# prequel-dev/plz4

Hardware: AMD Instinct MI355X
Metric: MiB/s enc+dec, 4MiB independent blocks, level 1, block-checksum on (duplex steps over 2 streams) (higher is better)
Workload: dtype u8

## Files before the change

plz4_amd/_native.py:

```python
from __future__ import annotations

import ctypes as C
import os

import numpy as np

HERE = os.path.dirname(os.path.abspath(__file__))
LIB_PATH = os.path.join(HERE, "libplz4hip.so")

ABI_VERSION = 2
SYMBOLS = [
    "plz4hip_abi_version", "plz4hip_device_count", "plz4hip_ctx_create", "plz4hip_ctx_destroy",
    "plz4hip_last_error", "plz4hip_compress_bound", "plz4hip_compress_batch", "plz4hip_decompress_batch",
    "plz4hip_xxh32_batch", "plz4hip_encode_records", "plz4hip_decode_records", "plz4hip_dev_stage_stride",
    "plz4hip_dev_encode_records", "plz4hip_dev_compact_records", "plz4hip_dev_scatter_records",
    "plz4hip_dev_decode_records", "plz4hip_dev_decode_records_ex", "plz4hip_dev_duplex_records", "plz4hip_dev_encode_body", "plz4hip_dev_duplex_body", "plz4hip_dev_encode_records_ex", "plz4hip_dev_encode_body_ex", "plz4hip_dev_compress", "plz4hip_dev_decompress", "plz4hip_ctx_trim",
    "plz4hip_ctx_counters",
    "plz4hip_dev_resident_waves", "plz4hip_dict_create", "plz4hip_dict_destroy", "plz4hip_compress_batch_dict", "plz4hip_decode_records_chains",
    "plz4hip_decompress_batch_dict", "plz4hip_encode_records_ex", "plz4hip_decode_records_ex",
    "plz4hip_xxh32_stream_create", "plz4hip_xxh32_stream_destroy", "plz4hip_xxh32_stream_reset", "plz4hip_xxh32_stream_update",
    "plz4hip_dev_xxh32_stream_update", "plz4hip_xxh32_stream_sum", "plz4hip_ctx_set_content_hash",
    "plz4hip_mgpu_create", "plz4hip_mgpu_destroy", "plz4hip_mgpu_count", "plz4hip_mgpu_ctx", "plz4hip_mgpu_last_error",
    "plz4hip_mgpu_compress_batch", "plz4hip_mgpu_decompress_batch", "plz4hip_mgpu_encode_records", "plz4hip_mgpu_decode_records",
    "plz4hip_mgpu_dev_encode_frame", "plz4hip_mgpu_dev_decode_frame",
# ... 408 lines not shown
        self._chk(self.L.plz4hip_dev_xxh32_stream_update(self.h, h, ptr, n, stream))

    def hash_sum(self, h) -> int:
        out = C.c_uint32()
        self._chk(self.L.plz4hip_xxh32_stream_sum(self.h, h, C.byref(out)))
        return int(out.value)

    def set_content_hash(self, h):
        self._chk(self.L.plz4hip_ctx_set_content_hash(self.h, h))

    def trim(self):
        self._chk(self.L.plz4hip_ctx_trim(self.h))

    COUNTERS = ("fx_blocks", "fx_rounds_last", "fx_pieces_again", "dx_blocks", "dxl_blocks", "dxl_rounds_last", "dxl_groups_last",
                "fxl_blocks", "l1x_blocks", "hcx_blocks", "dx_big_blocks", "dx_big_rounds_last", "dx_big_runs_last",
                "mx_blocks", "mx_rounds_last", "mx_pieces_again", "mxl_blocks", "hb_blocks", "hb_pieces_last")

    def counters(self) -> dict:
        out = (C.c_int64 * len(self.COUNTERS))()
        rc = int(self.L.plz4hip_ctx_counters(self.h, out, len(self.COUNTERS)))
        if rc < 0:
            self._chk(rc)
        return {k: int(out[i]) for i, k in enumerate(self.COUNTERS)}


class MultiEngine:

    def __init__(self, devices):
        self.L = load()
        arr = (C.c_int * len(devices))(*devices)
        h = C.c_void_p()
# ... 73 lines not shown
```

plz4_amd/csrc/plz4hip.hip:

```cpp
#include <hip/hip_runtime.h>

#include <array>
#include <atomic>
#include <mutex>
#include <thread>
#include <string>
#include <vector>
#include <cstdio>
#include <cstring>

#include "../../include/plz4hip.h"
#include "stream_ws.h"
#if defined(PLZ4_STATS)
__device__ unsigned long long plz4_stats[24];
#endif
#include "lz4_device.inl"
#include "lz4_seq_device.inl"
#include "lz4hc_device.inl"
#include "lz4hc12_device.inl"
#include "lz4hc_lists_device.inl"
#include "lz4hc_lazy_device.inl"
#include "lz4hcx_device.inl"
#include "lz4_dx_device.inl"
#include "lz4_fx_device.inl"
// ... 42 lines not shown
    int             h12Gather, h12Idle;
    SeqInfo*        l1Info;
    uint64_t*       l1Seq;      int64_t l1SeqStride;
    uint32_t*       l1ChunkBytes; uint32_t* l1ChunkOff; int l1MaxChunks;
    uint8_t*        l1Bk;
    int             l1MaxLen;
    int             lzSegs, lzMinSeg;
    uint64_t*       lzRec;      uint64_t* lzBridge;  int64_t lzRecStride;
    LzSegMeta*      lzMeta;     uint64_t* lzStarts;  LzPiece* lzPieces;
    uint64_t*       dxT;        int64_t dxTStride;
    uint32_t*       dxPtr;      int64_t dxPtrStride;
    DxUnit*         dxUnits;    int dxMaxSeg;   int dxRound;
    DxInfo*         dxInfo;
    int64_t*        bodyOff;    int64_t bodyCap;
    uint32_t*       gate;       uint32_t gateSeq;
    const int64_t*  dxSrcOff;   const int32_t* dxLen;
    int32_t*        dxHashBad;
    int32_t*        dxlFirst;   int32_t* dxlChain;   uint32_t* dxlMoved;   int32_t* dxlGood;   int dxlRounds;
    int32_t*        dxlDead;    int dxlBlk0;    int dxlGroup;   int dxlGroups;
    uint64_t*       dxbTG;      int64_t dxbTGStride;   DxbEntry* dxbEnt;   int dxbGroups;   int dxbG;
    DxRun*          dxbRuns;    int dxbRunRoom;   int dxbThr;   DxbInfo* dxbInfo;   int dxbRounds;
};

__device__ __forceinline__ int next_block(uint32_t* q)
{
    uint32_t v = 0;
    if ((threadIdx.x & 63u) == 0) v = atomicAdd(q, 1u);
    return (int)plz4_readfirstlane(v);
}

// ... 50 lines not shown
        const uint8_t* s = a.src + (int64_t)i * a.srcStride;
        encode_out(a, i, s, n, false, [&](uint8_t* out, int cap) { return wave_encode_block(s, n, out, cap, lds); });
    }
}

template <int kLdsWin = 0>
__device__ __forceinline__ void l1_parse_loop(const CodecArgs& a, uint32_t* lds, uint8_t* scr = nullptr)
{
    for (int i = next_block(a.queue); i < a.nBlocks; i = next_block(a.queue)) {
        const int gi = a.blk0 + i;
        const int n  = block_len(a, gi);
        int lastAnchor = 0, nseq = -1;
        if (n >= 0 && n <= a.l1MaxLen)
            nseq = wave_parse_l1<kLdsWin>(a.src + (int64_t)gi * a.srcStride, n, lds, a.l1Seq + (int64_t)i * a.l1SeqStride, &lastAnchor, scr);
        if ((threadIdx.x & 63u) == 0) { SeqInfo inf; inf.nseq = nseq; inf.lastAnchor = lastAnchor; inf.total = 0; inf.stored = 0; a.l1Info[i] = inf; }
    }
    if (a.gate && (threadIdx.x & 63u) == 0) atomicMax(a.gate, a.gateSeq);
}
__global__ __launch_bounds__(64) void k_parse_gate(const uint32_t* gate, uint32_t want)
{
    for (int it = 0; it < 400000; ++it) {
        if ((int32_t)(__hip_atomic_load(gate, __ATOMIC_RELAXED, __HIP_MEMORY_SCOPE_AGENT) - want) >= 0) break;
        __builtin_amdgcn_s_sleep(127);
    }
}
template <int W> __global__ __launch_bounds__(64 * W) void k_l1_parse(CodecArgs a)
{
    ENC_WAVE_TABLE(lds);
    l1_parse_loop<2>(a, lds);
}

template <bool kBack, bool kSeg = false> __device__ __forceinline__ void l1_sizes_body(const CodecArgs a, const FxlBlk* xb = nullptr)
{
    const int i = blockIdx.y, wave = blockIdx.x * 4 + (int)(threadIdx.x >> 6), nW = gridDim.x * 4;
    const int nseq = a.l1Info[i].nseq;
    if (nseq <= 0) return;
    const int gi = a.blk0 + i;
    const uint8_t*  s   = a.src + (int64_t)gi * a.srcStride;
    const uint64_t* seq = a.l1Seq + (int64_t)i * a.l1SeqStride;
    const int nChunks = (nseq + kSeqChunk - 1) / kSeqChunk;
    for (int c = wave; c < nChunks; c += nW) {
        const uint32_t v = seq_emit_sizes<kBack, kSeg>(s, seq, kBack ? a.l1Bk + (int64_t)i * a.l1SeqStride : nullptr, nseq, c, kSeg ? max_(xb[i].pfx, 0) : 0);
        if ((threadIdx.x & 63u) == 0) a.l1ChunkBytes[(int64_t)i * a.l1MaxChunks + c] = v;
    }
}
template <bool kBack> __global__ __launch_bounds__(256) void k_l1_sizes(CodecArgs a) { l1_sizes_body<kBack>(a); }

__global__ __launch_bounds__(256) void k_l1_scan(CodecArgs a)
{
    const int i = blockIdx.x * 4 + (int)(threadIdx.x >> 6);
    if (i >= a.nBlocks) return;
    const int gi = a.blk0 + i;
    const int n  = block_len(a, gi);
    SeqInfo inf = a.l1Info[i];
    const int cap = a.rawMode ? cap_of(a, gi) : a.bsz;
    int total = 0;
    const bool broken = inf.nseq == kSeqEngineFailed;
    if (inf.nseq >= 0)
        total = seq_emit_scan(a.l1ChunkBytes + (int64_t)i * a.l1MaxChunks, a.l1ChunkOff + (int64_t)i * a.l1MaxChunks, inf.nseq, inf.lastAnchor, n, cap);
    if ((threadIdx.x & 63u) == 0) {
        inf.total = total; inf.stored = (total == 0);
        a.l1Info[i] = inf;
        if (broken) a.result[gi] = PLZ4HIP_E_DEVICE;
        else if (a.rawMode) a.result[gi] = total;
// ... 24 lines not shown
    }
    if (kSeg && inf.nseq == kSeqElsewhere && inf.total > 0) {
        if (wave == 0) wave_copy(out, (const uint8_t*)(a.l1Seq + (int64_t)i * a.l1SeqStride), inf.total);
    } else if (inf.total > 0) {
        const uint64_t* seq = a.l1Seq + (int64_t)i * a.l1SeqStride;
        const int nChunks = (inf.nseq + kSeqChunk - 1) / kSeqChunk;
        for (int c = wave; c < (nChunks ? nChunks : 1); c += nW)
            seq_emit_write<kBack, kSeg>(s, n, seq, kBack ? a.l1Bk + (int64_t)i * a.l1SeqStride : nullptr, inf.nseq, inf.lastAnchor, c, nChunks ? a.l1ChunkOff[(int64_t)i * a.l1MaxChunks + c] : 0u, out,
                                        kSeg ? max_(xb[i].pfx, 0) : 0);
    } else if (!a.rawMode && n > 0) {
        const int slice = (((n + nW - 1) / nW) + 15) & ~15;
        const int off = wave * slice;
        if (off < n) wave_copy(out + off, s + off, min_(slice, n - off));
    }
}
template <bool kBack> __global__ __launch_bounds__(256) void k_l1_write(CodecArgs a) { l1_write_body<kBack>(a); }

__global__ __launch_bounds__(64) void k_l1_finish(CodecArgs a)
{
    const int i = blockIdx.x * 16 + (int)((threadIdx.x & 63u) >> 2);
    const uint8_t* p[1] = {nullptr};
    int n[1] = {-1};
    uint32_t x[1];
    int gi = 0;
    bool failed = false;
    if (i < a.nBlocks) {
        gi = a.blk0 + i;
        const SeqInfo inf = a.l1Info[i];
        const int c = inf.total ? inf.total : block_len(a, gi);
        failed = inf.nseq == kSeqEngineFailed;
        const uint8_t* rec = a.dst + (int64_t)gi * a.dstStride;
        bool written = true;
        if (a.bodyOff) {
            const int64_t off = a.bodyOff[gi];
// ... 1106 lines not shown
              offsetof(plz4hip_frame_index, status) == 56 && offsetof(plz4hip_frame_index, flags) == 52 && offsetof(plz4hip_frame_index, dictId) == 32,
              "plz4hip_frame_index is 64 bytes, as wave_store_frame lays it out");
static_assert(sizeof(StreamIndex) == sizeof(plz4hip_stream_index) && sizeof(StreamIndex) == 32 && offsetof(plz4hip_stream_index, flagsAnd) == 28 &&
              offsetof(StreamIndex, flagsAnd) == 28, "plz4hip_stream_index is 32 bytes");
__global__ __launch_bounds__(64) void k_index_stream(const uint8_t* bytes, int64_t nBytes, int maxFrames, int maxRecs, FrameIndex* frames,
                                                     int64_t* recOff, StreamIndex* info)
{
    wave_index_stream(bytes, nBytes, maxFrames, maxRecs, frames, recOff, info);
}

__global__ __launch_bounds__(64) void k_scan(const int32_t* __restrict__ len, int64_t* __restrict__ off, int n)
{
    wave_scan_lengths<false>(len, off, n, 1);
}

__global__ __launch_bounds__(64) void k_scan_from(const int32_t* __restrict__ len, int64_t* __restrict__ off, int n, int first)
{
    wave_scan_lengths<true>(len, off, n, first);
}

__global__ __launch_bounds__(256) void k_check_len(const int32_t* __restrict__ srcLen, int maxLen, int n, int32_t* __restrict__ lenOut, int32_t* __restrict__ result, int after)
{
    const int i = blockIdx.x * 256 + threadIdx.x;
    if (i >= n) return;
    const bool bad = srcLen[i] < 0 || srcLen[i] > maxLen;
    if (!after) lenOut[i] = bad ? 0 : srcLen[i];
    else if (bad) result[i] = PLZ4HIP_E_ARG;
}

__global__ __launch_bounds__(256) void k_out_len(const int32_t* __restrict__ res, int32_t* __restrict__ len, int n)
{
    const int i = blockIdx.x * 256 + threadIdx.x;
// ... 29 lines not shown
    int          qslot = 0;
    int          cus = 0;
    int          encWaves = 0, decWaves = 0;
    struct HostSlot { uint8_t* h = nullptr; size_t hcap = 0; uint8_t* d = nullptr; size_t dcap = 0; hipStream_t s = nullptr;
                      hipEvent_t evData = nullptr, evHash = nullptr; bool hashBusy = false; DeviceBuffer l1; };
    plz4hip_xxh32_stream* contentHash = nullptr;
    static constexpr int kSlots = 3;
    HostSlot     slot[kSlots];
    DeviceBuffer hc;  int hcWaves = 0;
    DeviceBuffer h12;  int h12ParseWaves = 0;  int h12SegWaves = 0;  int hcLazyWaves = 0;  size_t h12ErrOff = 0;
    StreamOrder  hcOrder;
    hipStream_t  hashStream = nullptr;
    static constexpr int kL1Shared = 2;
    DeviceBuffer l1[kL1Shared];  StreamOrder l1Order[kL1Shared];
    int          l1Refused = 0;
    uint32_t*    d_gate = nullptr; uint32_t gateSeq = 0; hipStream_t gateStream = nullptr; bool gatePending = false; int gateBlocks = 0;
    hipStream_t  hcBuildStream = nullptr; hipEvent_t evHcFork = nullptr, evHcHist = nullptr, evHcChain[2] = {nullptr, nullptr}, evHcFree[2] = {nullptr, nullptr};
    DeviceBuffer hcPfx;  int hcLazyExWaves = 0;
    DeviceBuffer hb;
    int hcxWaves[4] = {0, 0, 0, 0};
    DeviceBuffer dx;  StreamOrder dxOrder;
    hipStream_t  dxHashStream = nullptr; hipEvent_t evDxFork = nullptr, evDxHash = nullptr;
    DeviceBuffer fx;  StreamOrder fxOrder;
    DeviceBuffer mx;  StreamOrder mxOrder;
    DeviceBuffer xstage;  StreamOrder xstageOrder;
    static constexpr int kCounters = 19;
    unsigned long long* d_counters = nullptr;
    DeviceBuffer lenCopy;  StreamOrder lenOrder;
    DeviceBuffer chainCopy;  StreamOrder chainOrder;
    struct Owned { DeviceBuffer* buf; StreamOrder* order; bool trimmed; };
    std::array<Owned, 12> owned()
    {
        return {{{&hc, &hcOrder, true}, {&h12, &hcOrder, true}, {&hcPfx, &hcOrder, false}, {&l1[0], &l1Order[0], true},
                 {&l1[1], &l1Order[1], true}, {&dx, &dxOrder, true}, {&fx, &fxOrder, true}, {&lenCopy, &lenOrder, false},
                 {&chainCopy, &chainOrder, false}, {&xstage, &xstageOrder, true}, {&mx, &mxOrder, true}, {&hb, &hcOrder, true}}};
    }
};

struct plz4hip_xxh32_stream { XxhStream* d_state = nullptr; hipEvent_t done = nullptr; };

struct plz4hip_dict {
// ... 192 lines not shown
MxSwitches read_mx_switches() { return parse_mx_switches([](const char* n) { return (const char*)getenv(n); }); }
HcSwitches read_hc_switches() { return parse_hc_switches([](const char* n) { return (const char*)getenv(n); }); }
DxSwitches read_dx_switches() { return parse_dx_switches([](const char* n) { return (const char*)getenv(n); }); }

enum class Emit { Back, Mid, Seg };
void launch_emit(hipStream_t s, const CodecArgs& a, int ng, int g0, int maxChunks, Emit kind, const FxlBlk* xb = nullptr, bool ctxSmall = false)
{
    int wg = (16384 / ng) / 4;
    if (wg > (maxChunks + 3) / 4) wg = (maxChunks + 3) / 4;
    if (wg < 1) wg = 1;
    if (kind == Emit::Seg) hipLaunchKernelGGL(k_fxl_sizes, dim3(wg, ng), dim3(256), 0, s, a, xb);
    else if (kind == Emit::Mid) hipLaunchKernelGGL(k_l1_sizes<false>, dim3(wg, ng), dim3(256), 0, s, a);
    else hipLaunchKernelGGL(k_l1_sizes<true>, dim3(wg, ng), dim3(256), 0, s, a);
    hipLaunchKernelGGL(k_l1_scan, dim3((ng + 3) / 4), dim3(256), 0, s, a);
    if (ctxSmall && a.bodyOff) hipLaunchKernelGGL(k_fxl_small, dim3(ng < 1024 ? ng : 1024), dim3(64), 0, s, a);
    if (a.bodyOff) hipLaunchKernelGGL(k_scan_from, dim3(1), dim3(64), 0, s, (const int32_t*)(a.result + g0), a.bodyOff + g0, ng, g0 == 0 ? 1 : 0);
    if (kind == Emit::Seg) hipLaunchKernelGGL(k_fxl_write, dim3(wg, ng), dim3(256), 0, s, a, xb);
    else if (kind == Emit::Mid) hipLaunchKernelGGL(k_l1_write<false>, dim3(wg, ng), dim3(256), 0, s, a);
    else hipLaunchKernelGGL(k_l1_write<true>, dim3(wg, ng), dim3(256), 0, s, a);
    if (!a.rawMode && a.blockChecksum) hipLaunchKernelGGL(k_l1_finish, dim3((ng + 15) / 16), dim3(64), 0, s, a);
    if (ctxSmall && !a.bodyOff) hipLaunchKernelGGL(k_fxl_small, dim3(ng < 1024 ? ng : 1024), dim3(64), 0, s, a);
}

void launch_rec_verify(hipStream_t s, const CodecArgs& d)
{
    if (d.blockChecksum && d.nBlocks > 0) hipLaunchKernelGGL(k_rec_verify16, dim3((d.nBlocks + 15) / 16), dim3(64), 0, s, d);
}
int launch_l1(plz4hip_ctx* c, hipStream_t s, CodecArgs a, int nb, int maxLen, int rawMode, DeviceBuffer* ws, bool* midDeclined = nullptr,
              const CodecArgs* rider = nullptr, bool hist = false, bool l1x = false, const L1Switches* read = nullptr);

int launch_hc_body(plz4hip_ctx* c, hipStream_t s, const HcSwitches& sw, CodecArgs a, int nb, int maxLen, int rawMode, bool* forked);
// ... 243 lines not shown
        if (int rc = launch_l1(c, s, a, nb, maxLen, rawMode, nullptr, &declined)) return rc;
        if (!declined) return p.ctxBlocks ? hc_ctx_blocks(k, a) : PLZ4HIP_OK;
        a.hcPfx = nullptr;
        p = hc_route(shape, sw, true);
    }
    return p.route == HcRoute::Segmented ? hc_segmented(k, sw, p, a, forked) : hc_one_thread(k, sw, p, a);
}

void bind_l1(CodecArgs& a, uint8_t* base, const L1Layout& L)
{
    a.l1SeqStride = (int64_t)L.seqStride; a.l1MaxChunks = L.maxChunks;
    a.l1Info = (SeqInfo*)(base + L.offInfo);
    a.l1ChunkBytes = (uint32_t*)(base + L.offChunkBytes); a.l1ChunkOff = (uint32_t*)(base + L.offChunkOff);
    a.l1Seq = (uint64_t*)(base + L.offSeq); a.l1Bk = base + L.offBk;
}
FxlBlk* bind_pieces(PieceArgs& pc, uint8_t* base, const PieceLayout& L, bool hist)
{
    pc.meta = (PieceMeta*)(base + L.offMeta); pc.tabIn = (uint32_t*)(base + L.offIn); pc.tabOut = (uint32_t*)(base + L.offOut);
    pc.rec = (uint64_t*)(base + L.offRec);
    return hist ? (FxlBlk*)(base + L.offBlk) : nullptr;
}
template <class K> void launch_piece_rounds(hipStream_t s, const CodecArgs& a, const PieceArgs& pc, FxlBlk* xb, int ng, bool first)
{
    if (first) hipLaunchKernelGGL(k_piece_begin, dim3(1), dim3(64), 0, s, pc.cnt, (int)K::kRounds);
    if (K::kHist) hipLaunchKernelGGL(k_fxl_prep, dim3(ng), dim3(64), 0, s, a, pc, xb);
    for (int r = 1; r <= pc.P; ++r) hipLaunchKernelGGL(k_piece<K>, dim3(pc.P, ng), dim3(64), 0, s, a, pc, (const FxlBlk*)xb, r);
    hipLaunchKernelGGL(k_piece_gather<K>, dim3(pc.P, ng), dim3(64), 0, s, a, pc, (const FxlBlk*)xb);
}

int pick_l1_workspace(plz4hip_ctx* c, hipStream_t s, const L1Switches& sw)
// ... 41 lines not shown
              const CodecArgs* rider, bool hist, bool l1x, const L1Switches* read)
{
    hipError_t e;
    const L1Switches sw = read ? *read : read_l1_switches();
    const bool mid = midDeclined != nullptr;
    const L1Shape shape{nb, maxLen, rawMode != 0, mid, rider != nullptr, hist, l1x, a.bodyOff != nullptr, hist && a.dictLen >= 8};
    const L1Want want = l1_want(shape, sw);
    const bool mxl = mid && a.hcPfx != nullptr;
    const MxShape mxShape{a.level, nb, maxLen, a.hcEx != 0 || a.hcPfx != nullptr, rider != nullptr};
    const MxWant mxWant = !mid ? MxWant{} : mxl ? mxl_want(mxShape, read_mx_switches()) : mx_want(mxShape, read_mx_switches());
    a.rawMode = rawMode; a.blk0 = 0; a.nBlocks = nb;
    const bool shared = (ws == nullptr);
    int wsi = 0;
    if (shared) { wsi = pick_l1_workspace(c, s, sw); ws = &c->l1[wsi]; }
    bool granted = want.staged;
    const auto need_for = [&](int per) { return l1_layout(per, maxLen, l1x).total; };
    int per = nb;
    if (shared && granted && wsi != 0 && !ws->d && c->l1Refused > 0) { c->l1Refused--; wsi = 0; ws = &c->l1[0]; }
    if (shared && granted && wsi != 0 && !ws->d) {
        bool refused = false;  HIPCHK(c, ws->reserve(need_for(nb), c->l1Order[wsi], &refused));
        if (refused) {
            wsi = 0; ws = &c->l1[0]; c->l1Refused = 8;
            if (getenv("PLZ4HIP_VERBOSE")) fprintf(stderr, "plz4hip: level 1: no room for a second workspace of %zu MiB, sharing the first\n", need_for(nb) >> 20);
        }
    }
    StreamOrder* const order = shared ? &c->l1Order[wsi] : nullptr;
    if (granted && need_for(nb) > ws->bytes) {
        size_t freeB = 0, totalB = 0;
        if (hipMemGetInfo(&freeB, &totalB) != hipSuccess) return fail(c, PLZ4HIP_E_DEVICE, "hipMemGetInfo");
        int rc = PLZ4HIP_OK;
        const int64_t grp = l1_first_group(freeB, ws->bytes, sw.budgetGiB, sw.budgetMiB, l1_layout(1, maxLen, l1x).perBlock, nb);
// ... 2 lines not shown
            HIPCHK(c, order ? ws->reserve(need_for(per), *order, refused) : ws->reserve(need_for(per), s, refused));
            return (int)PLZ4HIP_OK;
        }, &rc);
        if (rc) return rc;
        if (!got) granted = false;
        if (getenv("PLZ4HIP_VERBOSE"))
            fprintf(stderr, "plz4hip: level 1, %d blocks of <= %d: free %zu MiB, workspace %zu MiB, groups of %d%s\n", nb, maxLen, freeB >> 20, ws->bytes >> 20, per, granted ? "" : " (fused)");
    }
    MarkOnExit job, pcJob;
    PieceArgs pc{};
    bool pcGranted = false;
    FxlBlk* xb = nullptr;
    L1Layout L{};
    if (granted) {
        if (order) { HIPCHK(c, order->wait(s)); job.arm(*order, s); }
        L = l1_layout(per, maxLen, l1x);
        a.l1MaxLen = maxLen;
        bind_l1(a, ws->d, L);
        const PieceCut cut = mid ? mxWant.cut() : want.cut();
        if (cut.on) {
            DeviceBuffer& buf = mid ? c->mx : c->fx;
            StreamOrder& ord = mid ? c->mxOrder : c->fxOrder;
            pc.pb = cut.piece; pc.warm = cut.warm; pc.P = cut.P; pc.recStride = piece_rec_stride(pc.pb); pc.cnt = c->d_counters;
            const bool blk = hist && !mid;
            const PieceLayout PL = piece_layout(per, pc.P, pc.recStride, mid ? kMxTab : kFxTab, blk);
            HIPCHK(c, ord.wait(s));
            bool refused = false;  HIPCHK(c, buf.reserve(PL.total, ord, &refused));
            if (!refused) { xb = bind_pieces(pc, buf.d, PL, blk); pcGranted = true; pcJob.arm(ord, s); }
        }
    }
    const L1Route route = l1_route(shape, sw, want, granted, pcGranted);
// ... 4 lines not shown
    case L1Route::MidDeclined:
        *midDeclined = true; return PLZ4HIP_OK;
    case L1Route::DictKernels: case L1Route::Fused:
        a.blk0 = 0; a.nBlocks = nb;
        a.queue = next_queue(c, s, &e); HIPCHK(c, e);
        if (route == L1Route::DictKernels) { if (rawMode) ENC_LAUNCH(k_encode_raw_dict, nb, c, s, a); else ENC_LAUNCH(k_encode_rec_dict, nb, c, s, a); }
        else                               { if (rawMode) ENC_LAUNCH(k_encode_raw, nb, c, s, a); else ENC_LAUNCH(k_encode_rec, nb, c, s, a); }
        if (route == L1Route::Fused && rider) { launch_rec_verify(s, *rider); hipLaunchKernelGGL(k_decode_rec, dim3(grid_for(rider->nBlocks, c->decWaves)), dim3(64), 0, s, *rider); }
        HIPCHK(c, hipGetLastError());
        HIPCHK(c, job.leave());
        HIPCHK(c, pcJob.leave());
        return PLZ4HIP_OK;
    default: break;
    }
    if (route == L1Route::L1x) xb = (FxlBlk*)(ws->d + L.offBlk);
    for (int g0 = 0; g0 < nb; g0 += per) {
        const int ng = nb - g0 < per ? nb - g0 : per;
        a.blk0 = g0; a.nBlocks = ng;
        a.queue = next_queue(c, s, &e); HIPCHK(c, e);
        if (rider && g0 == 0) launch_rec_verify(s, *rider);
        a.gate = nullptr;
        if (route == L1Route::Parse || route == L1Route::Duplex) {
            if (sw.noGate) c->gatePending = false;
            else if (int rc = l1_gate(c, s, a, ng)) return rc;
        } else if (route == L1Route::Mid) c->gatePending = false;
        switch (route) {
        case L1Route::Mid:
            if (mxOn && mxl) launch_piece_rounds<KMxl>(s, a, pc, xb, ng, g0 == 0);
            else if (mxOn) launch_piece_rounds<KMx>(s, a, pc, xb, ng, g0 == 0);
            else hipLaunchKernelGGL(hc_mid_kernel(a.hcPfx != nullptr), dim3(grid_for(ng, c->hcWaves)), dim3(64), 0, s, a);
            break;
        case L1Route::Fxl: launch_piece_rounds<KFxl>(s, a, pc, xb, ng, g0 == 0); break;
        case L1Route::Fx:  launch_piece_rounds<KFx>(s, a, pc, xb, ng, g0 == 0); break;
        case L1Route::L1x:
// ... 3 lines not shown
            if (route == L1Route::Duplex && g0 == 0) { if (int rc = launch_duplex(c, s, sw, a, *rider, ng)) return rc; break; }
#if defined(PLZ4_EXP_TABBITS)
            {
            int W = 10; if (const char* ev = getenv("PLZ4HIP_EXP_W")) W = atoi(ev);
#define EXP_CASE(WW) if (W == WW) { int per = 0; hipOccupancyMaxActiveBlocksPerMultiprocessor(&per, k_l1_parse<WW>, 64 * WW, 0); \
                if (getenv("PLZ4HIP_VERBOSE")) fprintf(stderr, "exp: W=%d workgroups per CU %d\n", WW, per); \
                int wgs = c->cus * per; if (wgs * WW > ng) wgs = (ng + WW - 1) / WW; \
                hipLaunchKernelGGL(k_l1_parse<WW>, dim3(wgs), dim3(64 * WW), 0, s, a); }
            EXP_CASE(4) EXP_CASE(5) EXP_CASE(6) EXP_CASE(8) EXP_CASE(9) EXP_CASE(10) EXP_CASE(12) EXP_CASE(13) EXP_CASE(14) EXP_CASE(16)
#undef EXP_CASE
            }
#else
            ENC_LAUNCH(k_l1_parse, ng, c, s, a);
#endif
        }
        launch_emit(s, a, ng, g0, L.maxChunks, hist ? Emit::Seg : mid ? Emit::Mid : Emit::Back, xb, shape.ctx);
        HIPCHK(c, hipGetLastError());
    }
    HIPCHK(c, job.leave());
    HIPCHK(c, pcJob.leave());
    return PLZ4HIP_OK;
}

template <class Layout> void bind_dx_tables(CodecArgs& a, uint8_t* base, const Layout& L)
{
    a.dxT = (uint64_t*)(base + L.offT); a.dxTStride = (int64_t)L.tStride;
    a.dxPtr = (uint32_t*)(base + L.offPtr); a.dxPtrStride = (int64_t)L.pStride;
    a.dxUnits = (DxUnit*)(base + L.offUnits); a.dxMaxSeg = L.maxSeg;
    a.dxInfo = (DxInfo*)(base + L.offInfo);
}
void bind_dx(CodecArgs& a, uint8_t* base, const DxLayout& L, bool records, bool hashed, bool hist)
// ... 237 lines not shown
void plz4hip_ctx_destroy(plz4hip_ctx* c)
{
    if (!c) return;
    DeviceGuard dg(c->device);
    for (auto& w : c->owned()) (void)w.buf->release(*w.order);
    for (auto& w : c->owned()) w.order->destroy();
    if (c->stream) { hipStreamSynchronize(c->stream); hipStreamDestroy(c->stream); }
    for (auto& sl : c->slot) {
        if (sl.s) { hipStreamSynchronize(sl.s); hipStreamDestroy(sl.s); }
        if (sl.evData) hipEventDestroy(sl.evData);
        if (sl.evHash) hipEventDestroy(sl.evHash);
        if (sl.h) hipHostFree(sl.h);
        if (sl.d) hipFree(sl.d);
        sl.l1.release();
    }
    for (hipEvent_t ev : {c->evDxFork, c->evDxHash}) if (ev) hipEventDestroy(ev);
    if (c->hashStream) { hipStreamSynchronize(c->hashStream); hipStreamDestroy(c->hashStream); }
    if (c->hcBuildStream) { hipStreamSynchronize(c->hcBuildStream); hipStreamDestroy(c->hcBuildStream); }
    for (void* p : {(void*)c->d_queues, (void*)c->d_gate, (void*)c->d_counters}) if (p) hipFree(p);
    for (hipEvent_t ev : {c->evHcFork, c->evHcHist, c->evHcChain[0], c->evHcChain[1], c->evHcFree[0], c->evHcFree[1]}) if (ev) hipEventDestroy(ev);
    delete c;
}

int plz4hip_ctx_trim(plz4hip_ctx* c)
{
    if (!c) return PLZ4HIP_E_ARG;
    std::lock_guard<std::mutex> g(c->mu);
    ENTER_DEVICE(c);
    for (auto& sl : c->slot) {
        if (sl.s) HIPCHK(c, hipStreamSynchronize(sl.s));
        if (sl.h) { hipHostFree(sl.h); sl.h = nullptr; sl.hcap = 0; }
// ... 822 lines not shown
```

plz4_amd/csrc/route.h:

```cpp
#pragma once
#include <climits>
#include <cstdio>
#include <cstdlib>
#include <vector>

namespace plz4 {

constexpr int kUnset = INT_MIN;

struct PieceCut { bool on; int piece, warm, P; };
inline PieceCut piece_cut(bool on, int maxLen, int pieceKiB, int warmKiB)
{
    PieceCut c{};
    c.on = on;
    if (on) { c.piece = pieceKiB << 10; c.warm = warmKiB << 10; c.P = (maxLen + c.piece - 1) / c.piece; }
    return c;
}
template <class Get> void parse_piece_kib(Get&& get, const char* pieceName, const char* warmName, int* pieceKiB, int* warmKiB)
{
    if (const char* v = get(pieceName)) { const int x = (int)atol(v); if (x >= 1 && x <= 4096) *pieceKiB = x; }
    if (const char* v = get(warmName)) { const int x = (int)atol(v); if (x >= 0 && x <= 4096) *warmKiB = x; }
}

constexpr int  kFxMaxBlocks = 128;
constexpr bool kL1xDefault = true;
struct L1Switches {
    bool fused = false;
    int  fxLinked = kUnset;
    int  fxMax = kFxMaxBlocks;
    int  fxPieceKiB = 64, fxWarmKiB = 64;
    int  l1x = kUnset;
    bool oneWorkspace = false;
    long budgetGiB = 0, budgetMiB = 0;
    bool noGate = false;
    int  duplexP = 1, duplexD = 1, duplexPrio = 3;
};

inline bool fxl_wanted(const L1Switches& sw, int nb, int maxLen)
{
    if (sw.fxLinked == 0) return false;
    return nb <= sw.fxMax && maxLen >= kFxMinLen && maxLen <= kSeqMaxBlock && !sw.fused;
}
inline bool l1x_on(const L1Switches& sw) { return !sw.fused && (sw.l1x == kUnset ? kL1xDefault : sw.l1x != 0); }

enum class L1Route { Fused, DictKernels, Parse, Duplex, Mid, Fx, Fxl, L1x, MidDeclined, NoMemBody };
struct L1Shape { int nb, maxLen; bool raw, mid, rider, hist, l1x, body, ctx; };
struct L1Want { bool staged, fx; int piece, warm, P; PieceCut cut() const { return PieceCut{fx, piece, warm, P}; } };
inline L1Want l1_want(const L1Shape& k, const L1Switches& sw)
{
    L1Want w{};
    const bool inRange = k.maxLen > 0 && k.maxLen <= kSeqMaxBlock && !sw.fused;
// ... 200 lines not shown
}

template <class Get> L1Switches parse_l1_switches(Get&& get)
{
    const auto num = [&](const char* n, long unset) { const char* v = get(n); return v ? atol(v) : unset; };
    L1Switches sw;
    sw.fused = get("PLZ4HIP_L1_FUSED") != nullptr;
    sw.fxLinked = (int)num("PLZ4HIP_FX_LINKED", kUnset);
    if (const char* v = get("PLZ4HIP_FX_MAX_BLOCKS")) sw.fxMax = atoi(v);
    parse_piece_kib(get, "PLZ4HIP_FX_PIECE_KIB", "PLZ4HIP_FX_WARMUP_KIB", &sw.fxPieceKiB, &sw.fxWarmKiB);
    sw.l1x = (int)num("PLZ4HIP_L1X", kUnset);
    sw.oneWorkspace = num("PLZ4HIP_L1_WORKSPACES", 0) == 1;
    sw.budgetGiB = num("PLZ4HIP_L1_BUDGET_GIB", 0);
    sw.budgetMiB = num("PLZ4HIP_L1_BUDGET_MIB", 0);
    sw.noGate = get("PLZ4HIP_EXP_NO_GATE") != nullptr;
    if (const char* v = get("PLZ4HIP_DUPLEX")) { if (sscanf(v, "%d,%d", &sw.duplexP, &sw.duplexD) != 2) { sw.duplexP = 1; sw.duplexD = 1; } }
    sw.duplexPrio = (int)num("PLZ4HIP_DUPLEX_PRIO", 3);
    return sw;
}
template <class Get> HcSwitches parse_hc_switches(Get&& get)
{
    const auto num = [&](const char* n, long unset) { const char* v = get(n); return v ? atol(v) : unset; };
    const auto set = [&](const char* n) { return get(n) != nullptr; };
    HcSwitches sw;
    sw.hcx = (int)num("PLZ4HIP_HCX", kUnset);
    sw.extOff = set("PLZ4HIP_HC_EXT_OFF"); sw.midOff = set("PLZ4HIP_HC_MID_OFF"); sw.lazyOff = set("PLZ4HIP_HC_LAZY_OFF");
    sw.preOff = set("PLZ4HIP_HC_PRE_OFF"); sw.listsOff = set("PLZ4HIP_HC_LISTS_OFF");
    sw.h12Off = set("PLZ4HIP_HC12_OFF"); sw.h12Lazy = set("PLZ4HIP_HC12_LAZY"); sw.h12SegOff = set("PLZ4HIP_HC12_SEG_OFF");
    { const int m = (int)num("PLZ4HIP_HC_MIN_SEG", 0); if (m >= 64) sw.minSeg = m; }
    { const int n = (int)num("PLZ4HIP_HC_SEGS", kLzMaxSegs); sw.segs = n < 1 ? 1 : (n > kLzMaxSegs ? kLzMaxSegs : n); }
// ... 37 lines not shown
```

plz4_amd/csrc/stream_ws.h:

```cpp
#pragma once

struct StreamOrder {
    hipEvent_t  done = nullptr;
    hipStream_t stream = nullptr;
    bool        pending = false;

    hipError_t wait(hipStream_t s) { return pending && stream != s ? hipStreamWaitEvent(s, done, 0) : hipSuccess; }
    hipError_t mark(hipStream_t s)
    {
        hipError_t e = done ? hipSuccess : hipEventCreateWithFlags(&done, hipEventDisableTiming);
        if (e == hipSuccess) e = hipEventRecord(done, s);
        if (e == hipSuccess) { pending = true; stream = s; }
        return e;
    }
    hipError_t drain()
    {
        const hipError_t e = pending ? hipEventSynchronize(done) : hipSuccess;
        if (e == hipSuccess) pending = false;
        return e;
    }
    bool idle()
    {
        if (!pending || hipEventQuery(done) == hipSuccess) return true;
        (void)hipGetLastError();
// ... 5 lines not shown
        if (done) hipEventDestroy(done);
        done = nullptr; stream = nullptr; pending = false;
    }
};

struct MarkOnExit {
    StreamOrder* order = nullptr;
    hipStream_t  s = nullptr;
    MarkOnExit() = default;
    MarkOnExit(const MarkOnExit&) = delete;
    void arm(StreamOrder& o, hipStream_t st) { order = &o; s = st; }
    hipError_t leave() { StreamOrder* o = order; order = nullptr; return o ? o->mark(s) : hipSuccess; }
    ~MarkOnExit() { (void)leave(); }
};

struct DeviceBuffer {
    uint8_t* d = nullptr;
    size_t   bytes = 0;

    template <class Drain> hipError_t reserve_behind(size_t need, bool* refused, Drain&& drained)
    {
        *refused = false;
        if (need <= bytes) return hipSuccess;
        if (d) { const hipError_t e = drained(); if (e != hipSuccess) return e; }
        release();
        if (hipMalloc((void**)&d, need) != hipSuccess) { (void)hipGetLastError(); d = nullptr; *refused = true; }
        else bytes = need;
        return hipSuccess;
    }
    hipError_t reserve(size_t need, StreamOrder& o, bool* refused) { return reserve_behind(need, refused, [&] { return o.drain(); }); }
// ... 5 lines not shown
```

plz4_amd/csrc/ws_layout.h:

```cpp
#pragma once
#include <vector>

namespace plz4 {

inline size_t round_up(size_t v, size_t a) { return (v + a - 1) / a * a; }

struct WsTake { size_t off, count, size, align; };
struct Carver {
    std::vector<WsTake>* log = nullptr;
    size_t at = 0, perBlock = 0;
    template <class T> size_t take(size_t count, size_t align = 256)
    {
        const size_t off = at;
        at = off + round_up(count * sizeof(T), align);
        if (log) log->push_back({off, count, sizeof(T), alignof(T)});
        return off;
    }
    template <class T> size_t per_block(size_t blocks, size_t each, size_t align = 256)
    {
        perBlock += each * sizeof(T);
        return take<T>(blocks * each, align);
    }
};

// ... 28 lines not shown
    if (group >= 1) grp = group;
    if (grp < 1) grp = 1;
    return grp > nb ? nb : grp;
}

inline int64_t l1_first_group(size_t freeB, size_t held, long budgetGiB, long budgetMiB, size_t perBlock, int nb)
{
    size_t budget = (freeB + held) / 2;
    if (budgetGiB >= 1) budget = (size_t)budgetGiB << 30;
    if (budgetMiB >= 1) budget = (size_t)budgetMiB << 20;
    if (budget < held) budget = held;
    const int64_t grp = (int64_t)(budget / (perBlock + 64));
    return grp > nb ? nb : grp;
}

struct L1Layout { size_t seqStride; int maxChunks; size_t perBlock, offInfo, offChunkBytes, offChunkOff, offSeq, offBk, offBlk, total; };
inline L1Layout l1_layout(int per, int maxLen, bool l1x, std::vector<WsTake>* log = nullptr)
{
    L1Layout L{};
    L.seqStride = round_up((size_t)(maxLen > 0 ? maxLen : 0) / 4 + 3, 64);
    L.maxChunks = (int)((L.seqStride + kSeqChunk - 1) / kSeqChunk);
    Carver c{log};
    const size_t n = (size_t)per;
    L.offInfo = c.per_block<SeqInfo>(n, 1);
    L.offChunkBytes = c.per_block<uint32_t>(n, (size_t)L.maxChunks);
    L.offChunkOff = c.per_block<uint32_t>(n, (size_t)L.maxChunks);
    L.offSeq = c.per_block<uint64_t>(n, L.seqStride, 8);
    L.offBk = c.per_block<uint8_t>(n, L.seqStride, 8);
    if (l1x) L.offBlk = c.per_block<FxlBlk>(n, 1, 1);
    L.perBlock = c.perBlock; L.total = c.at;
    return L;
}

struct PieceLayout { size_t offMeta, offIn, offOut, offRec, offBlk, total; };
inline PieceLayout piece_layout(int per, int P, int recStride, int tabWords, bool hist, std::vector<WsTake>* log = nullptr)
{
    PieceLayout L{};
    Carver c{log};
    const size_t nP = (size_t)per * (size_t)P;
    L.offMeta = c.take<PieceMeta>(nP);
    L.offIn = c.take<uint32_t>(nP * (size_t)tabWords, 4);
    L.offOut = c.take<uint32_t>(2 * nP * (size_t)tabWords, 4);
    L.offRec = c.take<uint64_t>(nP * (size_t)recStride, 8);
    L.offBlk = c.at;
// ... 172 lines not shown
```

Measured before the change: 92910.

## Overlap L1 emit with parse via sliced early-emit on a side stream

Parse kernel now bumps per-slice completion counters. A side stream runs gate kernels that poll these counters and, once a slice is fully parsed, launches the emit chain (sizes/scan/write/finish) for that slice. Each slice also gets a fallback emit on the main stream that runs only when its gate timed out. The goal is to overlap the emit phase with the tail of parsing. In exchange it adds a memset, events, polling kernels that occupy CUs, and more kernel launches per step, and it makes ordering depend on atomics and fences.

Result: no change. 93240, median of 6 (+0.4%).

```diff
diff --git a/plz4_amd/_native.py b/plz4_amd/_native.py
--- a/plz4_amd/_native.py
+++ b/plz4_amd/_native.py
@@ -446,7 +446,8 @@
 
     COUNTERS = ("fx_blocks", "fx_rounds_last", "fx_pieces_again", "dx_blocks", "dxl_blocks", "dxl_rounds_last", "dxl_groups_last",
                 "fxl_blocks", "l1x_blocks", "hcx_blocks", "dx_big_blocks", "dx_big_rounds_last", "dx_big_runs_last",
-                "mx_blocks", "mx_rounds_last", "mx_pieces_again", "mxl_blocks", "hb_blocks", "hb_pieces_last")
+                "mx_blocks", "mx_rounds_last", "mx_pieces_again", "mxl_blocks", "hb_blocks", "hb_pieces_last",
+                "early_emit_slices", "late_emit_slices")
 
     def counters(self) -> dict:
         out = (C.c_int64 * len(self.COUNTERS))()
diff --git a/plz4_amd/csrc/plz4hip.hip b/plz4_amd/csrc/plz4hip.hip
--- a/plz4_amd/csrc/plz4hip.hip
+++ b/plz4_amd/csrc/plz4hip.hip
@@ -80,6 +80,8 @@
     DxInfo*         dxInfo;
     int64_t*        bodyOff;    int64_t bodyCap;
     uint32_t*       gate;       uint32_t gateSeq;
+    uint32_t*       sliceDone;  int sliceBlocks;
+    const uint32_t* runIf;      uint32_t runWant;
     const int64_t*  dxSrcOff;   const int32_t* dxLen;
     int32_t*        dxHashBad;
     int32_t*        dxlFirst;   int32_t* dxlChain;   uint32_t* dxlMoved;   int32_t* dxlGood;   int dxlRounds;
@@ -160,6 +162,14 @@
         if (n >= 0 && n <= a.l1MaxLen)
             nseq = wave_parse_l1<kLdsWin>(a.src + (int64_t)gi * a.srcStride, n, lds, a.l1Seq + (int64_t)i * a.l1SeqStride, &lastAnchor, scr);
         if ((threadIdx.x & 63u) == 0) { SeqInfo inf; inf.nseq = nseq; inf.lastAnchor = lastAnchor; inf.total = 0; inf.stored = 0; a.l1Info[i] = inf; }
+        if (a.sliceDone) {
+            __asm__ volatile("s_waitcnt vmcnt(0)" ::: "memory");
+            if ((threadIdx.x & 63u) == 0) {
+                __builtin_amdgcn_fence(__ATOMIC_RELEASE, "agent");
+                __asm__ volatile("s_waitcnt vmcnt(0)" ::: "memory");
+                __hip_atomic_fetch_add(a.sliceDone + i / a.sliceBlocks, 1u, __ATOMIC_RELAXED, __HIP_MEMORY_SCOPE_AGENT);
+            }
+        }
     }
     if (a.gate && (threadIdx.x & 63u) == 0) atomicMax(a.gate, a.gateSeq);
 }
@@ -170,6 +180,25 @@
         __builtin_amdgcn_s_sleep(127);
     }
 }
+__global__ __launch_bounds__(64) void k_slice_gate(const uint32_t* done, uint32_t want, const uint32_t* prevState, uint32_t* state, int polls,
+                                                   unsigned long long* cnt)
+{
+    const bool first = prevState == nullptr;
+    const uint32_t prev = first ? 1u : __hip_atomic_load(prevState, __ATOMIC_RELAXED, __HIP_MEMORY_SCOPE_AGENT);
+    bool ok = false;
+    for (int it = 0; it < polls && prev == 1u; ++it) {
+        ok = slice_gate_ok(__hip_atomic_load(done, __ATOMIC_RELAXED, __HIP_MEMORY_SCOPE_AGENT), want, first, prev);
+        if (ok) break;
+        __builtin_amdgcn_s_sleep(127);
+    }
+    if (ok) __builtin_amdgcn_fence(__ATOMIC_ACQUIRE, "agent");
+    if ((threadIdx.x & 63u) == 0) {
+        if (ok) *state = 1u;
+        atomicAdd(cnt + (ok ? 0 : 1), 1ull);
+    }
+}
+__device__ __forceinline__ bool run_if(const uint32_t* runIf, uint32_t runWant) { return !runIf || *runIf == runWant; }
+
 template <int W> __global__ __launch_bounds__(64 * W) void k_l1_parse(CodecArgs a)
 {
     ENC_WAVE_TABLE(lds);
@@ -190,10 +219,15 @@
         if ((threadIdx.x & 63u) == 0) a.l1ChunkBytes[(int64_t)i * a.l1MaxChunks + c] = v;
     }
 }
-template <bool kBack> __global__ __launch_bounds__(256) void k_l1_sizes(CodecArgs a) { l1_sizes_body<kBack>(a); }
+template <bool kBack> __global__ __launch_bounds__(256) void k_l1_sizes(CodecArgs a)
+{
+    if constexpr (kBack) { if (!run_if(a.runIf, a.runWant)) return; }
+    l1_sizes_body<kBack>(a);
+}
 
 __global__ __launch_bounds__(256) void k_l1_scan(CodecArgs a)
 {
+    if (!run_if(a.runIf, a.runWant)) return;
     const int i = blockIdx.x * 4 + (int)(threadIdx.x >> 6);
     if (i >= a.nBlocks) return;
     const int gi = a.blk0 + i;
@@ -248,10 +282,15 @@
         if (off < n) wave_copy(out + off, s + off, min_(slice, n - off));
     }
 }
-template <bool kBack> __global__ __launch_bounds__(256) void k_l1_write(CodecArgs a) { l1_write_body<kBack>(a); }
+template <bool kBack> __global__ __launch_bounds__(256) void k_l1_write(CodecArgs a)
+{
+    if constexpr (kBack) { if (!run_if(a.runIf, a.runWant)) return; }
+    l1_write_body<kBack>(a);
+}
 
 __global__ __launch_bounds__(64) void k_l1_finish(CodecArgs a)
 {
+    if (!run_if(a.runIf, a.runWant)) return;
     const int i = blockIdx.x * 16 + (int)((threadIdx.x & 63u) >> 2);
     const uint8_t* p[1] = {nullptr};
     int n[1] = {-1};
@@ -1388,8 +1427,10 @@
     wave_scan_lengths<false>(len, off, n, 1);
 }
 
-__global__ __launch_bounds__(64) void k_scan_from(const int32_t* __restrict__ len, int64_t* __restrict__ off, int n, int first)
-{
+__global__ __launch_bounds__(64) void k_scan_from(const int32_t* __restrict__ len, int64_t* __restrict__ off, int n, int first,
+                                                  const uint32_t* runIf, uint32_t runWant)
+{
+    if (!run_if(runIf, runWant)) return;
     wave_scan_lengths<true>(len, off, n, first);
 }
 
@@ -1449,6 +1490,7 @@
     static constexpr int kL1Shared = 2;
     DeviceBuffer l1[kL1Shared];  StreamOrder l1Order[kL1Shared];
     int          l1Refused = 0;
+    hipEvent_t   evEeFork[kL1Shared] = {nullptr, nullptr}, evEeJoin[kL1Shared] = {nullptr, nullptr};
     uint32_t*    d_gate = nullptr; uint32_t gateSeq = 0; hipStream_t gateStream = nullptr; bool gatePending = false; int gateBlocks = 0;
     hipStream_t  hcBuildStream = nullptr; hipEvent_t evHcFork = nullptr, evHcHist = nullptr, evHcChain[2] = {nullptr, nullptr}, evHcFree[2] = {nullptr, nullptr};
     DeviceBuffer hcPfx;  int hcLazyExWaves = 0;
@@ -1459,7 +1501,7 @@
     DeviceBuffer fx;  StreamOrder fxOrder;
     DeviceBuffer mx;  StreamOrder mxOrder;
     DeviceBuffer xstage;  StreamOrder xstageOrder;
-    static constexpr int kCounters = 19;
+    static constexpr int kCounters = 21;  static constexpr int kCntEarlySlices = 19;
     unsigned long long* d_counters = nullptr;
     DeviceBuffer lenCopy;  StreamOrder lenOrder;
     DeviceBuffer chainCopy;  StreamOrder chainOrder;
@@ -1682,7 +1724,7 @@
     else hipLaunchKernelGGL(k_l1_sizes<true>, dim3(wg, ng), dim3(256), 0, s, a);
     hipLaunchKernelGGL(k_l1_scan, dim3((ng + 3) / 4), dim3(256), 0, s, a);
     if (ctxSmall && a.bodyOff) hipLaunchKernelGGL(k_fxl_small, dim3(ng < 1024 ? ng : 1024), dim3(64), 0, s, a);
-    if (a.bodyOff) hipLaunchKernelGGL(k_scan_from, dim3(1), dim3(64), 0, s, (const int32_t*)(a.result + g0), a.bodyOff + g0, ng, g0 == 0 ? 1 : 0);
+    if (a.bodyOff) hipLaunchKernelGGL(k_scan_from, dim3(1), dim3(64), 0, s, (const int32_t*)(a.result + g0), a.bodyOff + g0, ng, g0 == 0 ? 1 : 0, a.runIf, a.runWant);
     if (kind == Emit::Seg) hipLaunchKernelGGL(k_fxl_write, dim3(wg, ng), dim3(256), 0, s, a, xb);
     else if (kind == Emit::Mid) hipLaunchKernelGGL(k_l1_write<false>, dim3(wg, ng), dim3(256), 0, s, a);
     else hipLaunchKernelGGL(k_l1_write<true>, dim3(wg, ng), dim3(256), 0, s, a);
@@ -1956,6 +1998,16 @@
     a.l1ChunkBytes = (uint32_t*)(base + L.offChunkBytes); a.l1ChunkOff = (uint32_t*)(base + L.offChunkOff);
     a.l1Seq = (uint64_t*)(base + L.offSeq); a.l1Bk = base + L.offBk;
 }
+CodecArgs slice_l1(const CodecArgs& a, int e0, int e1, const uint32_t* runIf, uint32_t runWant)
+{
+    CodecArgs x = a;
+    x.l1Info += e0;
+    x.l1Seq += (int64_t)e0 * a.l1SeqStride; x.l1Bk += (int64_t)e0 * a.l1SeqStride;
+    x.l1ChunkBytes += (int64_t)e0 * a.l1MaxChunks; x.l1ChunkOff += (int64_t)e0 * a.l1MaxChunks;
+    x.blk0 += e0; x.nBlocks = e1 - e0;
+    x.runIf = runIf; x.runWant = runWant;
+    return x;
+}
 FxlBlk* bind_pieces(PieceArgs& pc, uint8_t* base, const PieceLayout& L, bool hist)
 {
     pc.meta = (PieceMeta*)(base + L.offMeta); pc.tabIn = (uint32_t*)(base + L.offIn); pc.tabOut = (uint32_t*)(base + L.offOut);
@@ -2027,7 +2079,8 @@
     int wsi = 0;
     if (shared) { wsi = pick_l1_workspace(c, s, sw); ws = &c->l1[wsi]; }
     bool granted = want.staged;
-    const auto need_for = [&](int per) { return l1_layout(per, maxLen, l1x).total; };
+    const int sliceWords = shared ? kEarlyEmitMaxSlices : 0;
+    const auto need_for = [&](int per) { return l1_layout(per, maxLen, l1x, nullptr, sliceWords).total; };
     int per = nb;
     if (shared && granted && wsi != 0 && !ws->d && c->l1Refused > 0) { c->l1Refused--; wsi = 0; ws = &c->l1[0]; }
     if (shared && granted && wsi != 0 && !ws->d) {
@@ -2060,7 +2113,7 @@
     L1Layout L{};
     if (granted) {
         if (order) { HIPCHK(c, order->wait(s)); job.arm(*order, s); }
-        L = l1_layout(per, maxLen, l1x);
+        L = l1_layout(per, maxLen, l1x, nullptr, sliceWords);
         a.l1MaxLen = maxLen;
         bind_l1(a, ws->d, L);
         const PieceCut cut = mid ? mxWant.cut() : want.cut();
@@ -2095,10 +2148,24 @@
     default: break;
     }
     if (route == L1Route::L1x) xb = (FxlBlk*)(ws->d + L.offBlk);
+    const bool eeRoute = (route == L1Route::Parse || route == L1Route::Duplex) && shared && per == nb && !sw.gateProbe;
+    const EarlyEmitPlan ee = eeRoute ? early_emit_plan(nb, sw.earlyMinBlocks == kUnset ? 8 * c->cus : sw.earlyMinBlocks, early_emit_slices(sw, c->gatePending && c->gateStream != s)) : EarlyEmitPlan{0, 0, nb};
+    uint32_t* const sliceDone = ee.on() ? (uint32_t*)(ws->d + L.offSliceDone) : nullptr;
+    uint32_t* const sliceState = ee.on() ? (uint32_t*)(ws->d + L.offSliceState) : nullptr;
+    JoinOnExit join;
+    a.sliceDone = nullptr; a.runIf = nullptr;
     for (int g0 = 0; g0 < nb; g0 += per) {
         const int ng = nb - g0 < per ? nb - g0 : per;
         a.blk0 = g0; a.nBlocks = ng;
         a.queue = next_queue(c, s, &e); HIPCHK(c, e);
+        if (ee.on()) {
+            static_assert(sizeof(uint32_t) * kEarlyEmitMaxSlices <= 256, "sliceDone and sliceState: one take of 256 bytes each");
+            HIPCHK(c, hipMemsetAsync(sliceDone, 0, (size_t)((uint8_t*)(sliceState + kEarlyEmitMaxSlices) - (uint8_t*)sliceDone), s));
+            for (hipEvent_t* ev : {&c->evEeFork[wsi], &c->evEeJoin[wsi]}) if (!*ev) HIPCHK(c, hipEventCreateWithFlags(ev, hipEventDisableTiming));
+            HIPCHK(c, hipEventRecord(c->evEeFork[wsi], s));
+            join.arm(c->stream, c->evEeJoin[wsi], s);
+            a.sliceDone = sliceDone; a.sliceBlocks = ee.sliceBlocks;
+        }
         if (rider && g0 == 0) launch_rec_verify(s, *rider);
         a.gate = nullptr;
         if (route == L1Route::Parse || route == L1Route::Duplex) {
@@ -2132,7 +2199,27 @@
             ENC_LAUNCH(k_l1_parse, ng, c, s, a);
 #endif
         }
-        launch_emit(s, a, ng, g0, L.maxChunks, hist ? Emit::Seg : mid ? Emit::Mid : Emit::Back, xb, shape.ctx);
+        if (sw.gateProbe && a.gate) {
+            hipLaunchKernelGGL(k_parse_gate, dim3(1), dim3(64), 0, c->stream, (const uint32_t*)a.gate, a.gateSeq);
+        }
+        if (ee.on()) {
+            const hipStream_t side = c->stream;
+            HIPCHK(c, hipStreamWaitEvent(side, c->evEeFork[wsi], 0));
+            a.sliceDone = nullptr;
+            for (int j = 0; j < ee.n; ++j) {
+                const int e0 = ee.bound(j), e1 = ee.bound(j + 1);
+                hipLaunchKernelGGL(k_slice_gate, dim3(1), dim3(64), 0, side, (const uint32_t*)(sliceDone + j), (uint32_t)(e1 - e0),
+                                   (const uint32_t*)(j ? sliceState + j - 1 : nullptr), sliceState + j, j < sw.earlyLateFrom ? sw.earlyPolls : 0,
+                                   c->d_counters + plz4hip_ctx::kCntEarlySlices);
+                launch_emit(side, slice_l1(a, e0, e1, sliceState + j, 1u), e1 - e0, e0, L.maxChunks, Emit::Back);
+            }
+            HIPCHK(c, join.leave());
+            for (int j = 0; j < ee.n; ++j) {
+                const int e0 = ee.bound(j), e1 = ee.bound(j + 1);
+                launch_emit(s, slice_l1(a, e0, e1, sliceState + j, 0u), e1 - e0, e0, L.maxChunks, Emit::Back);
+            }
+        } else
+            launch_emit(s, a, ng, g0, L.maxChunks, hist ? Emit::Seg : mid ? Emit::Mid : Emit::Back, xb, shape.ctx);
         HIPCHK(c, hipGetLastError());
     }
     HIPCHK(c, job.leave());
@@ -2400,7 +2487,7 @@
         if (sl.d) hipFree(sl.d);
         sl.l1.release();
     }
-    for (hipEvent_t ev : {c->evDxFork, c->evDxHash}) if (ev) hipEventDestroy(ev);
+    for (hipEvent_t ev : {c->evDxFork, c->evDxHash, c->evEeFork[0], c->evEeFork[1], c->evEeJoin[0], c->evEeJoin[1]}) if (ev) hipEventDestroy(ev);
     if (c->hashStream) { hipStreamSynchronize(c->hashStream); hipStreamDestroy(c->hashStream); }
     if (c->hcBuildStream) { hipStreamSynchronize(c->hcBuildStream); hipStreamDestroy(c->hcBuildStream); }
     for (void* p : {(void*)c->d_queues, (void*)c->d_gate, (void*)c->d_counters}) if (p) hipFree(p);
diff --git a/plz4_amd/csrc/route.h b/plz4_amd/csrc/route.h
--- a/plz4_amd/csrc/route.h
+++ b/plz4_amd/csrc/route.h
@@ -1,5 +1,6 @@
 #pragma once
 #include <climits>
+#include <cstdint>
 #include <cstdio>
 #include <cstdlib>
 #include <vector>
@@ -24,6 +25,9 @@
 
 constexpr int  kFxMaxBlocks = 128;
 constexpr bool kL1xDefault = true;
+constexpr int  kEarlyEmitDefault = 6;
+constexpr int  kEarlyEmitMaxSlices = 16;
+constexpr int  kSliceGatePolls = 400000;
 struct L1Switches {
     bool fused = false;
     int  fxLinked = kUnset;
@@ -33,8 +37,34 @@
     bool oneWorkspace = false;
     long budgetGiB = 0, budgetMiB = 0;
     bool noGate = false;
+    bool gateProbe = false;
     int  duplexP = 1, duplexD = 1, duplexPrio = 3;
-};
+    int  earlyEmit = kUnset;
+    int  earlyMinBlocks = kUnset;
+    int  earlyPolls = kSliceGatePolls;
+    int  earlyLateFrom = INT_MAX;
+};
+
+struct EarlyEmitPlan {
+    int n, sliceBlocks, nb;
+    bool on() const { return n > 0; }
+    int  bound(int j) const { const int64_t b = (int64_t)j * sliceBlocks; return b < nb ? (int)b : nb; }
+};
+inline EarlyEmitPlan early_emit_plan(int nb, int residentGate, int K)
+{
+    EarlyEmitPlan p{0, 0, nb};
+    if (K < 1 || nb < 1 || nb < residentGate) return p;
+    if (K > kEarlyEmitMaxSlices) K = kEarlyEmitMaxSlices;
+    if (K > nb) K = nb;
+    p.sliceBlocks = (nb + K - 1) / K;
+    p.n = (nb + p.sliceBlocks - 1) / p.sliceBlocks;
+    return p;
+}
+inline int early_emit_slices(const L1Switches& sw, bool otherStreamsLaunchPending)
+{
+    return sw.earlyEmit != kUnset ? sw.earlyEmit : (otherStreamsLaunchPending ? 0 : kEarlyEmitDefault);
+}
+constexpr bool slice_gate_ok(uint32_t done, uint32_t want, bool first, uint32_t prevState) { return done == want && (first || prevState == 1u); }
 
 inline bool fxl_wanted(const L1Switches& sw, int nb, int maxLen)
 {
@@ -265,6 +295,11 @@
     sw.budgetGiB = num("PLZ4HIP_L1_BUDGET_GIB", 0);
     sw.budgetMiB = num("PLZ4HIP_L1_BUDGET_MIB", 0);
     sw.noGate = get("PLZ4HIP_EXP_NO_GATE") != nullptr;
+    sw.gateProbe = num("PLZ4HIP_EXP_GATE_PROBE", 0) == 1;
+    if (get("PLZ4HIP_EARLY_EMIT")) { const long k = num("PLZ4HIP_EARLY_EMIT", 0); sw.earlyEmit = k < 0 ? 0 : (k > kEarlyEmitMaxSlices ? kEarlyEmitMaxSlices : (int)k); }
+    { const long m = num("PLZ4HIP_EARLY_EMIT_MIN_BLOCKS", 0); if (m >= 1) sw.earlyMinBlocks = m > INT_MAX ? INT_MAX : (int)m; }
+    { const long p = num("PLZ4HIP_EARLY_EMIT_POLLS", kSliceGatePolls); sw.earlyPolls = p < 0 ? 0 : (p > kSliceGatePolls ? kSliceGatePolls : (int)p); }
+    { const long j = num("PLZ4HIP_EARLY_EMIT_LATE_FROM", -1); if (j >= 0) sw.earlyLateFrom = j > INT_MAX ? INT_MAX : (int)j; }
     if (const char* v = get("PLZ4HIP_DUPLEX")) { if (sscanf(v, "%d,%d", &sw.duplexP, &sw.duplexD) != 2) { sw.duplexP = 1; sw.duplexD = 1; } }
     sw.duplexPrio = (int)num("PLZ4HIP_DUPLEX_PRIO", 3);
     return sw;
diff --git a/plz4_amd/csrc/stream_ws.h b/plz4_amd/csrc/stream_ws.h
--- a/plz4_amd/csrc/stream_ws.h
+++ b/plz4_amd/csrc/stream_ws.h
@@ -43,6 +43,22 @@
     ~MarkOnExit() { (void)leave(); }
 };
 
+struct JoinOnExit {
+    hipStream_t side = nullptr, s = nullptr;
+    hipEvent_t  ev = nullptr;
+    JoinOnExit() = default;
+    JoinOnExit(const JoinOnExit&) = delete;
+    void arm(hipStream_t sideStream, hipEvent_t join, hipStream_t st) { side = sideStream; ev = join; s = st; }
+    hipError_t leave()
+    {
+        hipEvent_t e = ev; ev = nullptr;
+        if (!e) return hipSuccess;
+        const hipError_t r = hipEventRecord(e, side);
+        return r == hipSuccess ? hipStreamWaitEvent(s, e, 0) : r;
+    }
+    ~JoinOnExit() { (void)leave(); }
+};
+
 struct DeviceBuffer {
     uint8_t* d = nullptr;
     size_t   bytes = 0;
diff --git a/plz4_amd/csrc/ws_layout.h b/plz4_amd/csrc/ws_layout.h
--- a/plz4_amd/csrc/ws_layout.h
+++ b/plz4_amd/csrc/ws_layout.h
@@ -66,8 +66,8 @@
     return grp > nb ? nb : grp;
 }
 
-struct L1Layout { size_t seqStride; int maxChunks; size_t perBlock, offInfo, offChunkBytes, offChunkOff, offSeq, offBk, offBlk, total; };
-inline L1Layout l1_layout(int per, int maxLen, bool l1x, std::vector<WsTake>* log = nullptr)
+struct L1Layout { size_t seqStride; int maxChunks; size_t perBlock, offInfo, offChunkBytes, offChunkOff, offSeq, offBk, offBlk, offSliceDone, offSliceState, total; };
+inline L1Layout l1_layout(int per, int maxLen, bool l1x, std::vector<WsTake>* log = nullptr, int slices = 0)
 {
     L1Layout L{};
     L.seqStride = round_up((size_t)(maxLen > 0 ? maxLen : 0) / 4 + 3, 64);
@@ -80,6 +80,10 @@
     L.offSeq = c.per_block<uint64_t>(n, L.seqStride, 8);
     L.offBk = c.per_block<uint8_t>(n, L.seqStride, 8);
     if (l1x) L.offBlk = c.per_block<FxlBlk>(n, 1, 1);
+    if (slices > 0) {
+        c.at = round_up(c.at, 256);
+        L.offSliceDone = c.take<uint32_t>((size_t)slices); L.offSliceState = c.take<uint32_t>((size_t)slices);
+    }
     L.perBlock = c.perBlock; L.total = c.at;
     return L;
 }
```
